# DefaultRui/VLN-VER

Measured on AMD Instinct MI355X. Metric: viewpoints/sec (multi-view->voxel fwd+bwd), vocc.py config, higher is better.
Workload: dtype bf16

## Files before the change

### vln-ver_amd/csrc/ver_common.h

```cpp
#pragma once
#include <hip/hip_runtime.h>
#include <stdint.h>
#include "../../include/ver_ops.h"

#define VER_WAVE 64

int ver_fail(int code, const char* fmt, ...);
int ver_check_launch(const char* what);
int ver_zero_async(void* ptr, size_t bytes, void* stream);

#define VER_REQUIRE(cond, code, ...)                     \
    do {                                                 \
        if (!(cond)) return ver_fail(code, __VA_ARGS__); \
    } while (0)

struct Bilinear {
    float w[4];
    int key[4];
    float gx[4];
    float gy[4];
    bool any;
};

template <bool GRAD>
// ... 109 lines not shown
```

### vln-ver_amd/csrc/ver_gemm.hip

```cpp
#include "ver_common.h"

namespace {
typedef __bf16 bf16x8 __attribute__((ext_vector_type(8)));
typedef float f32x16 __attribute__((ext_vector_type(16)));
typedef int i32x2 __attribute__((ext_vector_type(2)));
typedef int i32x4 __attribute__((ext_vector_type(4)));
typedef __attribute__((address_space(3))) void lds_void;

constexpr int kTile = 256;
constexpr int kStageBytes = 32768;
constexpr int kStages = 4;
constexpr int kLdsBytes = kStages * kStageBytes;

template <int OFF>
__device__ __forceinline__ i32x2 tr_read(int addr) {
    i32x2 v;
    asm volatile("ds_read_b64_tr_b16 %0, %1 offset:%2" : "=v"(v) : "v"(addr), "n"(OFF) : "memory");
    return v;
}
template <int OFF>
__device__ __forceinline__ i32x4 row_read(int addr) {
    i32x4 v;
    asm volatile("ds_read_b128 %0, %1 offset:%2" : "=v"(v) : "v"(addr), "n"(OFF) : "memory");
    return v;
// ... 12 lines not shown
    int CW, ncst;
    signed char kind[64], dz[64], dy[64], dx[64];
    signed char pl[64];
    long plane_elems;
};

struct GemmArgs {
    const __bf16* A;
    const __bf16* W;
    const float* bias;
    __bf16* C;
    long lda, ldw, ldc, M;
    int K, N, tiles_n, T, per_xcd;
    int S, Kc;
    float* ws;
    TapArgs t;
};

struct GemmLane {
    int offA0, offA1;
    int offB0, offB1;
    int voA, voW;
    int stepW;
    int stepA16;
    int dmaA, dmaW;
};

constexpr int kOutside = (int)0x80000000;
template <int L>
__device__ __forceinline__ int cell_off(const TapArgs& t, int b, int zl, int y, int x, int dz) {
// ... 57 lines not shown
            __builtin_amdgcn_raw_ptr_buffer_load_lds(rcst, (lds_void*)(dst + 1024), 16, tl.vo2, ch, 0, 0);
        } else {
            __builtin_amdgcn_raw_ptr_buffer_load_lds(ra, (lds_void*)dst, 16, tl.vo1, ch, 0, 0);
            __builtin_amdgcn_raw_ptr_buffer_load_lds(ra, (lds_void*)(dst + 1024), 16, tl.vo2, ch, 0, 0);
        }
        tl.ch = ch + 64;
        if (tl.ch == __builtin_amdgcn_readfirstlane(tl.seglen)) {
            tl.ch = 0;
            tl.tap = __builtin_amdgcn_readfirstlane(tl.tap) + 1;
            tap_offsets<IMPL>(t, tl, ra);
        }
    }
}


template <int ST, int IMPL>
__device__ __forceinline__ void phase(char* lds, f32x16 (&acc)[4][2], const GemmLane& c, __amdgpu_buffer_rsrc_t& ra,
                                      __amdgpu_buffer_rsrc_t rw, int& soA, int& soW, const TapArgs& t, TapLane& tl,
                                      __amdgpu_buffer_rsrc_t rcst) {
    constexpr int SB = (ST & 1) * kStageBytes;
    constexpr int UP = ST >= 2 ? 65536 : 0;
    const int a0 = c.offA0 + UP, a1 = c.offA1 + UP, b0 = c.offB0 + UP, b1 = c.offB1 + UP;
    i32x4 av[2][4];
    i32x2 bl[2][2], bh[2][2];
    av[0][0] = row_read<SB>(a0);
    av[0][1] = row_read<SB + 2048>(a0);
    bl[0][0] = tr_read<SB + 16384>(b0);
    bh[0][0] = tr_read<SB + 16384 + 512>(b0);
    bl[0][1] = tr_read<SB + 16384>(b1);
    bh[0][1] = tr_read<SB + 16384 + 512>(b1);
    av[0][2] = row_read<SB + 4096>(a0);
    av[0][3] = row_read<SB + 6144>(a0);
    av[1][0] = row_read<SB>(a1);
    av[1][1] = row_read<SB + 2048>(a1);
    bl[1][0] = tr_read<SB + 24576>(b0);
    bh[1][0] = tr_read<SB + 24576 + 512>(b0);
    bl[1][1] = tr_read<SB + 24576>(b1);
    bh[1][1] = tr_read<SB + 24576 + 512>(b1);
    av[1][2] = row_read<SB + 4096>(a1);
    av[1][3] = row_read<SB + 6144>(a1);
    constexpr int DS = ((ST + 2) % kStages) * kStageBytes;
    request_a<IMPL>(lds + DS + c.dmaA, c, ra, rcst, soA, t, tl);
    __builtin_amdgcn_raw_ptr_buffer_load_lds(rw, (lds_void*)(lds + DS + 16384 + c.dmaW), 16, c.voW, soW, 0, 0);
    __builtin_amdgcn_raw_ptr_buffer_load_lds(rw, (lds_void*)(lds + DS + 24576 + c.dmaW), 16, c.voW, soW + c.stepW, 0, 0);
    soW += 2 * c.stepW;
    asm volatile("s_waitcnt vmcnt(4)" ::: "memory");
    __builtin_amdgcn_s_barrier();
    asm volatile("s_waitcnt lgkmcnt(0)"
                 : "+v"(av[0][0]), "+v"(av[0][1]), "+v"(av[0][2]), "+v"(av[0][3]), "+v"(av[1][0]), "+v"(av[1][1]), "+v"(av[1][2]),
                   "+v"(av[1][3]), "+v"(bl[0][0]), "+v"(bh[0][0]), "+v"(bl[0][1]), "+v"(bh[0][1]), "+v"(bl[1][0]), "+v"(bh[1][0]),
                   "+v"(bl[1][1]), "+v"(bh[1][1])
                 :
                 : "memory");
    bf16x8 a[2][4], b[2][2];
#pragma unroll
    for (int u = 0; u < 2; ++u) {
#pragma unroll
        for (int i = 0; i < 4; ++i) a[u][i] = __builtin_bit_cast(bf16x8, av[u][i]);
        b[u][0] = frag(bl[u][0], bh[u][0]);
        b[u][1] = frag(bl[u][1], bh[u][1]);
    }
    __builtin_amdgcn_sched_barrier(0);
    __builtin_amdgcn_s_setprio(1);
#pragma unroll
    for (int u = 0; u < 2; ++u)
#pragma unroll
        for (int it = 0; it < 4; ++it)
#pragma unroll
            for (int jt = 0; jt < 2; ++jt)
                acc[it][jt] = __builtin_amdgcn_mfma_f32_32x32x16_bf16(a[u][it], b[u][jt], acc[it][jt], 0, 0, 0);
    __builtin_amdgcn_s_setprio(0);
    __builtin_amdgcn_sched_barrier(0);
    __builtin_amdgcn_s_barrier();
}

template <int IMPL>
__global__ __launch_bounds__(512) void k_gemm_nn(GemmArgs p) {
    extern __shared__ __attribute__((aligned(1024))) char lds[];
    const int tid = threadIdx.x, lane = tid & 63;
    const int wave = __builtin_amdgcn_readfirstlane(tid >> 6);
    const int wr = wave >> 2, wc = wave & 3;
    const int item = (int)(blockIdx.x & 7) * p.per_xcd + (int)(blockIdx.x >> 3);
    if ((int)(blockIdx.x >> 3) >= p.per_xcd || item >= p.T * p.S) return;
    const int split = item / p.T, tile = item - split * p.T;
    const int mt = tile / p.tiles_n, nt = tile - mt * p.tiles_n;
    const long row0 = (long)mt * kTile;
    const int k0 = split * p.Kc, klen = min(p.Kc, p.K - k0);
    const int nphase = klen / 32;

    const __bf16* ab = IMPL < 0 ? p.A + row0 * p.lda + k0 : p.t.lattice;
    const long abytes = IMPL < 0 ? ((p.M - row0 - 1) * p.lda + klen) * 2 : p.t.lattice_bytes;
    __amdgpu_buffer_rsrc_t ra = __builtin_amdgcn_make_buffer_rsrc((void*)ab, 0, (int)max(0L, min(abytes, 0xFFFFFFFFL)), 0x00020000);
    const __amdgpu_buffer_rsrc_t rcst = __builtin_amdgcn_make_buffer_rsrc((void*)(IMPL < 0 ? ab : p.t.cst), 0,
                                                                          (int)(IMPL < 0 ? 0L : max(0L, min(p.t.cst_bytes, 0x7FFFFFFFL))), 0x00020000);
    const __bf16* wb = p.W + (long)k0 * p.ldw + (long)nt * kTile;
    const long wbytes = ((long)(klen - 1) * p.ldw + p.N - (long)nt * kTile) * 2;
    const __amdgpu_buffer_rsrc_t rw = __builtin_amdgcn_make_buffer_rsrc((void*)wb, 0, (int)max(0L, min(wbytes, 0xFFFFFFFFL)), 0x00020000);
    GemmLane c;
    {
        const int prow = 32 * wave + (lane >> 2);
        const int pch = (lane & 3) ^ ((prow >> 2) & 3);
        c.voA = (int)(prow * p.lda * 2) + pch * 16;
        c.dmaA = wave * 2048;
        c.stepA16 = (int)(16 * p.lda * 2);
        const int wrow = lane >> 3, wch = (lane & 7) ^ (((wrow >> 1) & 1) << 2);
        c.voW = (int)(((8 * (wave >> 2) + wrow) * p.ldw + 64 * (wave & 3)) * 2) + wch * 16;
        c.stepW = (int)(16 * p.ldw * 2);
        c.dmaW = wave * 1024;
    }
    {
        const int lbase = (int)(uintptr_t)(__attribute__((address_space(3))) char*)lds;
        const int i = lane & 31, sw = (i >> 2) & 3;
        c.offA0 = lbase + (128 * wr + i) * 64 + (((lane >> 5) ^ sw) << 4);
        c.offA1 = c.offA0 ^ 32;
        const int q = lane >> 4, cl = lane & 15;
        const int lowch = (2 * (q & 1) + ((cl & 3) >> 1)) ^ (((cl >> 3) & 1) << 2);
        c.offB0 = lbase + ((q >> 1) * 32 + (cl >> 2)) * 128 + lowch * 16 + (cl & 1) * 8 + wc * 1024;
        c.offB1 = c.offB0 ^ 64;
    }
    TapLane tl = {};
    if constexpr (IMPL >= 0) {
        const int prow = 32 * wave + (lane >> 2);
        const int hw = p.t.H * p.t.W;
        auto decode = [&](long r, int& b, int& zl, int& y, int& x) {
            if (r >= p.M) {
                b = -1, zl = y = x = 0;
                return;
            }
            b = (int)(r / p.t.P);
            const int pos = (int)(r - (long)b * p.t.P);
            zl = pos / hw;
            const int rem = pos - zl * hw;
            y = rem / p.t.W;
            x = rem - y * p.t.W;
        };
        decode(row0 + prow, tl.b1, tl.zl1, tl.y1, tl.x1);
        decode(row0 + prow + 16, tl.b2, tl.zl2, tl.y2, tl.x2);
        tl.pos1 = (tl.zl1 * p.t.H + tl.y1) * p.t.W + tl.x1;
        tl.pos2 = (tl.zl2 * p.t.H + tl.y2) * p.t.W + tl.x2;
        tl.chunk = ((lane & 3) ^ ((prow >> 2) & 3)) * 16;
        tl.tap = 0, tl.ch = 0;
        tap_offsets<IMPL>(p.t, tl, ra);
    }
    f32x16 acc[4][2];
#pragma unroll
    for (int it = 0; it < 4; ++it)
#pragma unroll
        for (int jt = 0; jt < 2; ++jt)
#pragma unroll
            for (int r = 0; r < 16; ++r) acc[it][jt][r] = 0.0f;

    int soA = 0, soW = 0;
#pragma unroll
    for (int s = 0; s < 2; ++s) {
        request_a<IMPL>(lds + s * kStageBytes + c.dmaA, c, ra, rcst, soA, p.t, tl);
        __builtin_amdgcn_raw_ptr_buffer_load_lds(rw, (lds_void*)(lds + s * kStageBytes + 16384 + c.dmaW), 16, c.voW, soW, 0, 0);
        __builtin_amdgcn_raw_ptr_buffer_load_lds(rw, (lds_void*)(lds + s * kStageBytes + 24576 + c.dmaW), 16, c.voW, soW + c.stepW, 0, 0);
        soW += 2 * c.stepW;
    }
    asm volatile("s_waitcnt vmcnt(4)" ::: "memory");
    __builtin_amdgcn_s_barrier();
    if (wr == 1) __builtin_amdgcn_s_barrier();

    int s = 0;
    for (; s + kStages <= nphase; s += kStages) {
        phase<0, IMPL>(lds, acc, c, ra, rw, soA, soW, p.t, tl, rcst);
        phase<1, IMPL>(lds, acc, c, ra, rw, soA, soW, p.t, tl, rcst);
        phase<2, IMPL>(lds, acc, c, ra, rw, soA, soW, p.t, tl, rcst);
        phase<3, IMPL>(lds, acc, c, ra, rw, soA, soW, p.t, tl, rcst);
    }
    const int rem = nphase - s;
    if (rem > 0) phase<0, IMPL>(lds, acc, c, ra, rw, soA, soW, p.t, tl, rcst);
    if (rem > 1) phase<1, IMPL>(lds, acc, c, ra, rw, soA, soW, p.t, tl, rcst);
    if (rem > 2) phase<2, IMPL>(lds, acc, c, ra, rw, soA, soW, p.t, tl, rcst);
    if (wr == 0) __builtin_amdgcn_s_barrier();
    asm volatile("s_waitcnt vmcnt(0)" ::: "memory");

    if (p.S > 1) {
        float* out = p.ws + (long)split * p.M * p.N;
        const long i0 = row0 + 128 * wr + 4 * (lane >> 5);
        const int j0 = nt * kTile + 64 * wc + (lane & 31);
#pragma unroll
        for (int it = 0; it < 4; ++it)
#pragma unroll
            for (int jt = 0; jt < 2; ++jt) {
                const int j = j0 + 32 * jt;
#pragma unroll
                for (int r = 0; r < 16; ++r) {
                    const long i = i0 + 32 * it + (r & 3) + 8 * (r >> 2);
                    if (i < p.M && j < p.N) out[i * p.N + j] = acc[it][jt][r];
                }
            }
        return;
    }
    __bf16* cb = p.C + row0 * p.ldc + (long)nt * kTile;
    const long cbytes = ((p.M - row0 - 1) * p.ldc + p.N - (long)nt * kTile) * 2;
    const __amdgpu_buffer_rsrc_t rc = __builtin_amdgcn_make_buffer_rsrc((void*)cb, 0, (int)max(0L, min(cbytes, 0xFFFFFFFFL)), 0x00020000);
    const int ldc2 = (int)(p.ldc * 2);
    const int vbase = (128 * wr + 4 * (lane >> 5)) * ldc2 + (64 * wc + (lane & 31)) * 2;
    const bool haspos = IMPL >= 0 && p.t.rowpos != nullptr;
    const int pos0 = haspos ? (int)((row0 + 128 * wr + 4 * (lane >> 5)) % p.t.P) : 0;
#pragma unroll
    for (int jt = 0; jt < 2; ++jt) {
        const int j = nt * kTile + 64 * wc + 32 * jt + (lane & 31);
        const float bj = (p.bias && j < p.N) ? p.bias[j] : 0.0f;
        const int vo = j < p.N ? vbase + 64 * jt : -2;
#pragma unroll
        for (int it = 0; it < 4; ++it) {
            float add[16];
#pragma unroll
            for (int r = 0; r < 16; ++r) {
                add[r] = bj;
                if (haspos) {
                    int pp = pos0 + 32 * it + (r & 3) + 8 * (r >> 2);
                    while (pp >= p.t.P) pp -= p.t.P;
                    const long row = row0 + 128 * wr + 4 * (lane >> 5) + 32 * it + (r & 3) + 8 * (r >> 2);
                    if (j < p.N && row < p.M) add[r] += p.t.rowpos[(long)pp * p.N + j];
                }
            }
#pragma unroll
            for (int r = 0; r < 16; ++r) {
                const __bf16 v = (__bf16)(acc[it][jt][r] + add[r]);
                __builtin_amdgcn_raw_buffer_store_b16(__builtin_bit_cast(short, v), rc, vo, (32 * it + (r & 3) + 8 * (r >> 2)) * ldc2, 0);
            }
        }
    }
}
__global__ __launch_bounds__(256) void k_gemm_reduce(const float* __restrict__ ws, const float* __restrict__ bias,
                                                     __bf16* __restrict__ c, long ldc, int S, long M, int N) {
    const long n4 = M * N / 4;
    const long stride = M * N;
    for (long e = blockIdx.x * 256L + threadIdx.x; e < n4; e += (long)gridDim.x * 256) {
        float4 acc = *reinterpret_cast<const float4*>(ws + 4 * e);
        for (int s = 1; s < S; ++s) {
            const float4 v = *reinterpret_cast<const float4*>(ws + s * stride + 4 * e);
            acc.x += v.x, acc.y += v.y, acc.z += v.z, acc.w += v.w;
        }
        const long i = (4 * e) / N;
        const int j = (int)(4 * e - i * N);
        if (bias) acc.x += bias[j], acc.y += bias[j + 1], acc.z += bias[j + 2], acc.w += bias[j + 3];
        typedef __bf16 bf16x4 __attribute__((ext_vector_type(4)));
// ... 49 lines not shown
    p.W = (const __bf16*)w;
    p.bias = bias;
    p.C = (__bf16*)c;
    p.lda = lda;
    p.ldw = ldw;
    p.ldc = ldc;
    p.M = M;
    p.K = K;
    p.N = N;
    p.tiles_n = (N + kTile - 1) / kTile;
    p.T = (int)((M + kTile - 1) / kTile) * p.tiles_n;
    p.Kc = splits == 1 ? K : ((K + splits - 1) / splits + 31) / 32 * 32;
    p.S = splits == 1 ? 1 : (K + p.Kc - 1) / p.Kc;
    p.ws = (float*)workspace;
    p.per_xcd = (p.T * p.S + 7) / 8;
    p.t = TapArgs{};
    hipError_t e = hipFuncSetAttribute((const void*)k_gemm_nn<-1>, hipFuncAttributeMaxDynamicSharedMemorySize, kLdsBytes);
    if (e != hipSuccess) return ver_fail(VER_ELAUNCH, "ver_gemm_nn: LDS attribute: %s", hipGetErrorString(e));
    hipLaunchKernelGGL(k_gemm_nn<-1>, dim3((unsigned)(8 * p.per_xcd)), dim3(512), kLdsBytes, st, p);
    if (p.S > 1) {
        long grid = (M * N / 4 + 255) / 256;
        if (grid > 4096) grid = 4096;
        hipLaunchKernelGGL(k_gemm_reduce, dim3((unsigned)grid), dim3(256), 0, st, (const float*)workspace, bias, (__bf16*)c, ldc, p.S, M, N);
    }
    return ver_check_launch("ver_gemm_nn");
}

extern "C" int ver_gemm_nn_segments(const void* lattice, int layout, int B, int H, int W, int C, const int* taps, int ntaps,
                                    const void* cst, int ncst, int cw, const void* w, long ldw, const float* rowpos,
                                    const float* bias, void* c, long ldc, int N, void* stream);
// ... 46 lines not shown
    p.W = (const __bf16*)w;
    p.bias = bias;
    p.C = (__bf16*)c;
    p.lda = 0;
    p.ldw = ldw;
    p.ldc = ldc;
    p.M = M;
    p.K = (int)K;
    p.N = N;
    p.tiles_n = (N + kTile - 1) / kTile;
    p.T = (int)((M + kTile - 1) / kTile) * p.tiles_n;
    p.Kc = (int)K;
    p.S = 1;
    p.ws = nullptr;
    p.per_xcd = (p.T + 7) / 8;
    p.t = TapArgs{};
    p.t.lattice = (const __bf16*)lattice;
    p.t.lattice_bytes = lbytes;
    p.t.B = B, p.t.H = H, p.t.W = W, p.t.C = C, p.t.ntaps = ntaps, p.t.P = 2 * H * W;
    p.t.rowpos = rowpos;
    VER_REQUIRE((plane_elems == 0) == (tap_plane == nullptr) && plane_elems >= 0 && (plane_elems == 0 || (nplanes > 0 && nplanes <= 64 &&
                plane_elems % 8 == 0)), VER_EINVAL, "ver_gemm_nn_planes: plane_elems, nplanes and tap_plane come together");
    p.t.plane_elems = plane_elems;
    for (int i = 0; i < ntaps; ++i) {
        VER_REQUIRE(!tap_plane || (tap_plane[i] >= 0 && tap_plane[i] < nplanes), VER_EINVAL, "ver_gemm_nn_planes: tap %d reads plane %d of %d", i,
                    tap_plane ? tap_plane[i] : 0, nplanes);
        p.t.pl[i] = (signed char)(tap_plane ? tap_plane[i] : 0);
    }
    p.t.cst = (const __bf16*)cst;
    p.t.cst_bytes = cst ? (long)2 * H * W * ncst * cw * 2 : 0;
// ... 25 lines not shown
```

### vln-ver_amd/csrc/ver_wgrad.hip

```cpp
#include <cstdlib>
#include "ver_common.h"

namespace {
typedef __bf16 bf16x8 __attribute__((ext_vector_type(8)));
typedef float f32x16 __attribute__((ext_vector_type(16)));
typedef short s16x4 __attribute__((ext_vector_type(4)));
typedef short s16x8 __attribute__((ext_vector_type(8)));
typedef __attribute__((address_space(3))) s16x4 lds_s16x4;
typedef __attribute__((address_space(3))) void lds_void;

constexpr int kTile = 256;
constexpr int kSlabRows = 16;
constexpr int kSlabBytes = 2 * kSlabRows * kTile * 2;
constexpr int kRing = 8;
constexpr int kLdsBytes = kRing * kSlabBytes;

typedef int i32x2 __attribute__((ext_vector_type(2)));
typedef int i32x4 __attribute__((ext_vector_type(4)));

template <int OFF>
__device__ __forceinline__ i32x2 tr_read(int addr) {
    i32x2 v;
    asm volatile("ds_read_b64_tr_b16 %0, %1 offset:%2" : "=v"(v) : "v"(addr), "n"(OFF) : "memory");
    return v;
// ... 5 lines not shown
struct WgradArgs {
    const __bf16* A;
    const __bf16* G;
    float* ws;
    long lda, ldg, M, Mc;
    int S, Ka, N, tiles_n, T;
    void* out;
    long ldo;
    int out_bf16;
    const __bf16* lattice;
    long lattice_bytes;
    const __bf16* cst;
    long cst_bytes;
    int B, H, W, C, P, CW, ncst, nseg;
    int seg_start[65];
    signed char kind[64], dz[64], dy[64], dx[64];
};

constexpr int kOutsideW = (int)0x80000000;
template <int L>
__device__ __forceinline__ int wcell_off(const WgradArgs& t, int b, int zl, int y, int x, int dz) {
    if ((unsigned)y >= (unsigned)t.H || (unsigned)x >= (unsigned)t.W) return kOutsideW;
    const int j = dz >> 1;
    int v;
    if (L == 0)
        v = ((b * 4 + zl + dz) * t.H + y) * t.W + x;
    else if (L == 2)
        v = ((((b * 2 + zl) * t.H + y) * t.W + x) << 1) + j;
    else
        v = (((((((y & 1) << 1 | (x & 1)) * t.B + b) * 2 + zl) * (t.H >> 1) + (y >> 1)) * (t.W >> 1) + (x >> 1)) << 1) + j;
// ... 30 lines not shown
    tl.boff += tl.pend;
    tl.rows_left -= kSlabRows;
    tl.vo = tl.rows_left > 0 ? (int)((unsigned)tfetched + (unsigned)tl.boff) : kOutsideW;
    tl.taddr += 4 * kSlabRows;
    tl.pend = 0;
    if (tl.taddr >= tl.tend) tl.taddr -= 4 * t.P, tl.pend = tl.bstep;
}

struct WgradLane {
    int offA0, offA1, offB0, offB1;
    int voA, voG;
    int stepA, stepG;
    int dmaoff;
};

template <int SLOT>
__device__ __forceinline__ void read_slab(const WgradLane& c, i32x2 (&al)[4], i32x2 (&ah)[4], i32x2 (&bl)[2], i32x2 (&bh)[2]) {
    constexpr int SB = (SLOT & 3) * kSlabBytes;
    constexpr int UP = SLOT >= 4 ? 65536 : 0;
    const int a0 = c.offA0 + UP, a1 = c.offA1 + UP, b0 = c.offB0 + UP, b1 = c.offB1 + UP;
    al[0] = tr_read<SB>(a0);
    ah[0] = tr_read<SB + 512>(a0);
    bl[0] = tr_read<SB>(b0);
    bh[0] = tr_read<SB + 512>(b0);
    al[1] = tr_read<SB>(a1);
    ah[1] = tr_read<SB + 512>(a1);
    bl[1] = tr_read<SB>(b1);
    bh[1] = tr_read<SB + 512>(b1);
    al[2] = tr_read<SB + 1024>(a0);
    ah[2] = tr_read<SB + 1536>(a0);
    al[3] = tr_read<SB + 1024>(a1);
    ah[3] = tr_read<SB + 1536>(a1);
}

template <int PS, int KP, int PF, int IMPL>
__device__ __forceinline__ void phase(char* lds, f32x16 (&acc)[4][2], const WgradLane& c, __amdgpu_buffer_rsrc_t ra,
                                      __amdgpu_buffer_rsrc_t rg, unsigned& soA, unsigned& soG, const WgradArgs& t, WTapLane& tl) {
    i32x2 al[KP][4], ah[KP][4], bl[KP][2], bh[KP][2];
    int tnext = 0;
    read_slab<PS * KP>(c, al[0], ah[0], bl[0], bh[0]);
    if constexpr (KP == 2) read_slab<PS * KP + 1>(c, al[KP - 1], ah[KP - 1], bl[KP - 1], bh[KP - 1]);
#pragma unroll
    for (int u = 0; u < KP; ++u) {
        const int ds = (PS * KP + u + PF) % kRing;
        if constexpr (IMPL < 0) {
            __builtin_amdgcn_raw_ptr_buffer_load_lds(ra, (lds_void*)(lds + ds * kSlabBytes + c.dmaoff), 16, c.voA, (int)soA, 0, 0);
        } else {
            static_assert(IMPL < 0 || KP == 1, "implicit A: one slab per phase");
            __builtin_amdgcn_raw_ptr_buffer_load_lds(ra, (lds_void*)(lds + ds * kSlabBytes + c.dmaoff), 16, tl.vo, 0, 0, 0);
            tnext = lds_read_b32(tl.taddr);
        }
        __builtin_amdgcn_raw_ptr_buffer_load_lds(rg, (lds_void*)(lds + ds * kSlabBytes + kSlabBytes / 2 + c.dmaoff), 16, c.voG, (int)soG, 0, 0);
        soA += (unsigned)c.stepA;
        soG += (unsigned)c.stepG;
    }
    asm volatile("s_waitcnt vmcnt(%0)" ::"n"(2 * (PF - KP)) : "memory");
    __builtin_amdgcn_s_barrier();
    asm volatile("s_waitcnt lgkmcnt(0)"
                 : "+v"(al[0][0]), "+v"(ah[0][0]), "+v"(al[0][1]), "+v"(ah[0][1]), "+v"(al[0][2]), "+v"(ah[0][2]), "+v"(al[0][3]),
                   "+v"(ah[0][3]), "+v"(bl[0][0]), "+v"(bh[0][0]), "+v"(bl[0][1]), "+v"(bh[0][1]), "+v"(tnext)
                 :
                 : "memory");

    if constexpr (KP == 2)
        asm volatile(""
                     : "+v"(al[KP - 1][0]), "+v"(ah[KP - 1][0]), "+v"(al[KP - 1][1]), "+v"(ah[KP - 1][1]), "+v"(al[KP - 1][2]),
                       "+v"(ah[KP - 1][2]), "+v"(al[KP - 1][3]), "+v"(ah[KP - 1][3]), "+v"(bl[KP - 1][0]), "+v"(bh[KP - 1][0]),
                       "+v"(bl[KP - 1][1]), "+v"(bh[KP - 1][1])
                     :
                     : "memory");
    bf16x8 a[KP][4], b[KP][2];
#pragma unroll
    for (int u = 0; u < KP; ++u) {
#pragma unroll
        for (int i = 0; i < 4; ++i) a[u][i] = frag(al[u][i], ah[u][i]);
        b[u][0] = frag(bl[u][0], bh[u][0]);
        b[u][1] = frag(bl[u][1], bh[u][1]);
    }
    __builtin_amdgcn_sched_barrier(0);
    __builtin_amdgcn_s_setprio(1);
#pragma unroll
    for (int u = 0; u < KP; ++u)
#pragma unroll
        for (int it = 0; it < 4; ++it)
#pragma unroll
            for (int jt = 0; jt < 2; ++jt)
                acc[it][jt] = __builtin_amdgcn_mfma_f32_32x32x16_bf16(a[u][it], b[u][jt], acc[it][jt], 0, 0, 0);
    __builtin_amdgcn_s_setprio(0);
    __builtin_amdgcn_sched_barrier(0);
    if constexpr (IMPL >= 0) {
        wtap_step(t, tl, tnext);
        __builtin_amdgcn_sched_barrier(0);
    }
    __builtin_amdgcn_s_barrier();
}

template <int PS, int KP, int PF, int IMPL>
__device__ __forceinline__ void phases_from(int left, char* lds, f32x16 (&acc)[4][2], const WgradLane& c,
                                            __amdgpu_buffer_rsrc_t ra, __amdgpu_buffer_rsrc_t rg, unsigned& soA, unsigned& soG,
                                            const WgradArgs& t, WTapLane& tl) {
    if constexpr (PS < kRing / KP) {
        if (left > PS * KP) {
            phase<PS, KP, PF, IMPL>(lds, acc, c, ra, rg, soA, soG, t, tl);
            phases_from<PS + 1, KP, PF, IMPL>(left, lds, acc, c, ra, rg, soA, soG, t, tl);
        }
    }
}

template <int KP, int PF, int IMPL>
__device__ __forceinline__ void wgrad_body(const WgradArgs& p) {
    static_assert(PF >= KP && PF + (KP == 1 ? 2 : 4) <= kRing, "prefetch distance against the ring (WAR on the slot)");
    extern __shared__ __attribute__((aligned(1024))) char lds[];
    const int tid = threadIdx.x, lane = tid & 63;
    const int wave = __builtin_amdgcn_readfirstlane(tid >> 6);
    const int wr = wave >> 2, wc = wave & 3;
    int chunk, tile;
    {
        const int b = blockIdx.x;
        if ((p.S & 7) == 0) {
            const int xcd = b & 7, idx = b >> 3;
            chunk = xcd + 8 * (idx / p.T);
            tile = idx % p.T;
        } else {
            chunk = b / p.T;
            tile = b % p.T;
        }
    }
    const int mt = tile / p.tiles_n, nt = tile - mt * p.tiles_n;
    const long row0 = (long)chunk * p.Mc;
    const long rows = max(0L, min(p.Mc, p.M - row0));
    const int nslab = (int)((rows + kSlabRows * KP - 1) / (kSlabRows * KP)) * KP;

    const __bf16* ab = IMPL < 0 ? p.A + row0 * p.lda + (long)mt * kTile : nullptr;
    const __bf16* gb = p.G + row0 * p.ldg + (long)nt * kTile;
    const long abytes = ((p.M - row0 - 1) * p.lda + p.Ka - (long)mt * kTile) * 2;
    const long gbytes = ((p.M - row0 - 1) * p.ldg + p.N - (long)nt * kTile) * 2;
    const __amdgpu_buffer_rsrc_t rg = __builtin_amdgcn_make_buffer_rsrc((void*)gb, 0, (int)max(0L, min(gbytes, 0xFFFFFFFFL)), 0x00020000);
    WgradLane c;
    const int prow = lane >> 3, pch = (lane & 7) ^ (((prow >> 1) & 1) << 2);
    WTapLane tl = {};
    bool a_cst = false;
    if constexpr (IMPL >= 0) {
// ... 29 lines not shown
        IMPL < 0 ? __builtin_amdgcn_make_buffer_rsrc((void*)ab, 0, (int)max(0L, min(abytes, 0xFFFFFFFFL)), 0x00020000)
                 : __builtin_amdgcn_make_buffer_rsrc((void*)(a_cst ? p.cst : p.lattice), 0,
                                                     (int)max(0L, min(a_cst ? p.cst_bytes : p.lattice_bytes, 0x7FFFFFFFL)), 0x00020000);
    c.voA = (int)(((8 * (wave >> 2) + prow) * p.lda + 64 * (wave & 3)) * 2) + pch * 16;
    c.voG = (int)(((8 * (wave >> 2) + prow) * p.ldg + 64 * (wave & 3)) * 2) + pch * 16;
    c.stepA = (int)(kSlabRows * p.lda * 2);
    c.stepG = (int)(kSlabRows * p.ldg * 2);
    c.dmaoff = wave * 1024;
    unsigned soA = 0, soG = 0;

    {
        const int q = lane >> 4, cl = lane & 15;
        const int lowch = (2 * (q & 1) + ((cl & 3) >> 1)) ^ (((cl >> 3) & 1) << 2);
        const int lbase = (int)(uintptr_t)(__attribute__((address_space(3))) char*)lds;
        const int rowoff = lbase + ((q >> 1) * 32 + (cl >> 2)) * 128 + lowch * 16 + (cl & 1) * 8;
        c.offA0 = rowoff + 2 * wr * 1024;
        c.offA1 = c.offA0 ^ 64;
        c.offB0 = rowoff + wc * 1024 + kSlabBytes / 2;
        c.offB1 = c.offB0 ^ 64;
    }

    f32x16 acc[4][2];
#pragma unroll
    for (int it = 0; it < 4; ++it)
#pragma unroll
        for (int jt = 0; jt < 2; ++jt)
#pragma unroll
            for (int r = 0; r < 16; ++r) acc[it][jt][r] = 0.0f;

#pragma unroll
    for (int s = 0; s < PF; ++s) {
        if constexpr (IMPL < 0) {
            __builtin_amdgcn_raw_ptr_buffer_load_lds(ra, (lds_void*)(lds + s * kSlabBytes + c.dmaoff), 16, c.voA, (int)soA, 0, 0);
        } else {
            __builtin_amdgcn_raw_ptr_buffer_load_lds(ra, (lds_void*)(lds + s * kSlabBytes + c.dmaoff), 16, tl.vo, 0, 0, 0);
            int tn = lds_read_b32(tl.taddr);
            asm volatile("s_waitcnt lgkmcnt(0)" : "+v"(tn)::"memory");
            wtap_step(p, tl, tn);
        }
        __builtin_amdgcn_raw_ptr_buffer_load_lds(rg, (lds_void*)(lds + s * kSlabBytes + kSlabBytes / 2 + c.dmaoff), 16, c.voG, (int)soG, 0, 0);
        soA += (unsigned)c.stepA;
        soG += (unsigned)c.stepG;
    }
    asm volatile("s_waitcnt vmcnt(%0)" ::"n"(2 * (PF - KP)) : "memory");
    __builtin_amdgcn_s_barrier();
    if (wr == 1) __builtin_amdgcn_s_barrier();

    int s = 0;
    for (; s + kRing <= nslab; s += kRing) phases_from<0, KP, PF, IMPL>(kRing, lds, acc, c, ra, rg, soA, soG, p, tl);
    phases_from<0, KP, PF, IMPL>(nslab - s, lds, acc, c, ra, rg, soA, soG, p, tl);
    if (wr == 0) __builtin_amdgcn_s_barrier();
    asm volatile("s_waitcnt vmcnt(0)" ::: "memory");

    const int i0 = mt * kTile + 128 * wr + 4 * (lane >> 5), j0 = nt * kTile + 64 * wc + (lane & 31);
    if (p.S == 1 && p.out) {
#pragma unroll
        for (int it = 0; it < 4; ++it)
#pragma unroll
            for (int jt = 0; jt < 2; ++jt) {
                const int j = j0 + 32 * jt;
#pragma unroll
                for (int r = 0; r < 16; ++r) {
                    const int i = i0 + 32 * it + (r & 3) + 8 * (r >> 2);
                    if (i < p.Ka && j < p.N) {
                        if (p.out_bf16)
                            reinterpret_cast<__bf16*>(p.out)[(long)i * p.ldo + j] = (__bf16)acc[it][jt][r];
                        else
                            reinterpret_cast<float*>(p.out)[(long)i * p.ldo + j] = acc[it][jt][r];
                    }
                }
            }
        return;
    }
    float* out = p.ws + (long)chunk * p.Ka * p.N;
#pragma unroll
    for (int it = 0; it < 4; ++it)
#pragma unroll
        for (int jt = 0; jt < 2; ++jt) {
            const int j = j0 + 32 * jt;
#pragma unroll
            for (int r = 0; r < 16; ++r) {
                const int i = i0 + 32 * it + (r & 3) + 8 * (r >> 2);
                if (i < p.Ka && j < p.N) out[(long)i * p.N + j] = acc[it][jt][r];
            }
        }
}

template <int KP, int PF>
__global__ __launch_bounds__(512) void k_wgrad_tn(WgradArgs p) {
    wgrad_body<KP, PF, -1>(p);
}

template <int L, int PF>
__global__ __launch_bounds__(512) void k_wgrad_tn_seg(WgradArgs p) {
    wgrad_body<1, PF, L>(p);
}

template <typename OT>
__global__ __launch_bounds__(256) void k_wgrad_reduce(const float* __restrict__ ws, OT* __restrict__ out, long ldo, int S,
                                                      int Ka, int N) {
    const long n4 = (long)Ka * N / 4;
    const long stride = (long)Ka * N;
    for (long e = blockIdx.x * 256L + threadIdx.x; e < n4; e += (long)gridDim.x * 256) {
        float4 acc = *reinterpret_cast<const float4*>(ws + 4 * e);
        for (int s = 1; s < S; ++s) {
            const float4 v = *reinterpret_cast<const float4*>(ws + s * stride + 4 * e);
            acc.x += v.x;
            acc.y += v.y;
            acc.z += v.z;
            acc.w += v.w;
// ... 111 lines not shown
    p.G = (const __bf16*)g;
    p.ws = (float*)workspace;
    p.lda = lda;
    p.ldg = ldg;
    p.M = M;
    p.Mc = Mc;
    p.S = S;
    p.Ka = Ka;
    p.N = N;
    p.tiles_n = (N + kTile - 1) / kTile;
    p.T = ((Ka + kTile - 1) / kTile) * p.tiles_n;
    const bool direct = S == 1 && M > 0;
    p.out = direct ? out : nullptr;
    p.ldo = ldo;
    p.out_bf16 = out_dtype == VER_BF16;
    hipError_t e = hipSuccess;
    if (M > 0) {
        switch (flags & 15) {
            case 4: launch_tn<1, 4>(p, p.T * S, st, e); break;
            case 5: launch_tn<1, 5>(p, p.T * S, st, e); break;
            case 6: launch_tn<1, 6>(p, p.T * S, st, e); break;
            case 8 + 2: launch_tn<2, 2>(p, p.T * S, st, e); break;
            case 8 + 4: launch_tn<2, 4>(p, p.T * S, st, e); break;
            default: launch_tn<1, 3>(p, p.T * S, st, e); break;
        }
        if (e != hipSuccess) return ver_fail(VER_ELAUNCH, "ver_wgrad_tn: LDS attribute: %s", hipGetErrorString(e));
    } else if (int zrc = ver_zero_async(workspace, (size_t)S * Ka * N * sizeof(float), st)) {
        return zrc;
    }
    if (direct) return ver_check_launch("ver_wgrad_tn");
// ... 103 lines not shown
```

Measured before the change: 701.8.

## Specialize GEMM and wgrad kernels for ragged edge tiles to skip dead MFMAs

Adds NIT-templated variants of the bf16 GEMM and weight-gradient tile bodies that compute only 1, 2 or 4 row sub-tiles per wave. Edge tiles with at most 64 valid columns or at most 128 valid rows now dispatch to the reduced variant, which drops LDS reads and MFMAs on padding. Wave-to-row and column mappings are remapped so the waves still cover the valid region. The path is on by default and can be turned off with VER_RAGGED_TILES=0. The cost is more kernel code paths, possible register and instruction-cache pressure, and waves that may sit idle or duplicate work in the reduced modes.

Measured after the change: 705.8 (median of 6 runs). No clear change (+0.6%).

```diff
diff --git a/vln-ver_amd/csrc/ver_common.h b/vln-ver_amd/csrc/ver_common.h
--- a/vln-ver_amd/csrc/ver_common.h
+++ b/vln-ver_amd/csrc/ver_common.h
@@ -1,6 +1,7 @@
 #pragma once
 #include <hip/hip_runtime.h>
 #include <stdint.h>
+#include <stdlib.h>
 #include "../../include/ver_ops.h"
 
 #define VER_WAVE 64
@@ -8,6 +9,11 @@
 int ver_fail(int code, const char* fmt, ...);
 int ver_check_launch(const char* what);
 int ver_zero_async(void* ptr, size_t bytes, void* stream);
+
+static inline int ver_ragged_tiles() {
+    const char* v = getenv("VER_RAGGED_TILES");
+    return !(v && v[0] == '0' && v[1] == 0);
+}
 
 #define VER_REQUIRE(cond, code, ...)                     \
     do {                                                 \
diff --git a/vln-ver_amd/csrc/ver_gemm.hip b/vln-ver_amd/csrc/ver_gemm.hip
--- a/vln-ver_amd/csrc/ver_gemm.hip
+++ b/vln-ver_amd/csrc/ver_gemm.hip
@@ -50,6 +50,7 @@
     int K, N, tiles_n, T, per_xcd;
     int S, Kc;
     float* ws;
+    int ragged;
     TapArgs t;
 };
 
@@ -137,31 +138,35 @@
 }
 
 
-template <int ST, int IMPL>
-__device__ __forceinline__ void phase(char* lds, f32x16 (&acc)[4][2], const GemmLane& c, __amdgpu_buffer_rsrc_t& ra,
+template <int ST, int IMPL, int NIT>
+__device__ __forceinline__ void phase(char* lds, f32x16 (&acc)[NIT][2], const GemmLane& c, __amdgpu_buffer_rsrc_t& ra,
                                       __amdgpu_buffer_rsrc_t rw, int& soA, int& soW, const TapArgs& t, TapLane& tl,
                                       __amdgpu_buffer_rsrc_t rcst) {
     constexpr int SB = (ST & 1) * kStageBytes;
     constexpr int UP = ST >= 2 ? 65536 : 0;
     const int a0 = c.offA0 + UP, a1 = c.offA1 + UP, b0 = c.offB0 + UP, b1 = c.offB1 + UP;
-    i32x4 av[2][4];
+    i32x4 av[2][NIT];
     i32x2 bl[2][2], bh[2][2];
     av[0][0] = row_read<SB>(a0);
-    av[0][1] = row_read<SB + 2048>(a0);
+    if constexpr (NIT >= 2) av[0][1] = row_read<SB + 2048>(a0);
     bl[0][0] = tr_read<SB + 16384>(b0);
     bh[0][0] = tr_read<SB + 16384 + 512>(b0);
     bl[0][1] = tr_read<SB + 16384>(b1);
     bh[0][1] = tr_read<SB + 16384 + 512>(b1);
-    av[0][2] = row_read<SB + 4096>(a0);
-    av[0][3] = row_read<SB + 6144>(a0);
+    if constexpr (NIT == 4) {
+        av[0][2] = row_read<SB + 4096>(a0);
+        av[0][3] = row_read<SB + 6144>(a0);
+    }
     av[1][0] = row_read<SB>(a1);
-    av[1][1] = row_read<SB + 2048>(a1);
+    if constexpr (NIT >= 2) av[1][1] = row_read<SB + 2048>(a1);
     bl[1][0] = tr_read<SB + 24576>(b0);
     bh[1][0] = tr_read<SB + 24576 + 512>(b0);
     bl[1][1] = tr_read<SB + 24576>(b1);
     bh[1][1] = tr_read<SB + 24576 + 512>(b1);
-    av[1][2] = row_read<SB + 4096>(a1);
-    av[1][3] = row_read<SB + 6144>(a1);
+    if constexpr (NIT == 4) {
+        av[1][2] = row_read<SB + 4096>(a1);
+        av[1][3] = row_read<SB + 6144>(a1);
+    }
     constexpr int DS = ((ST + 2) % kStages) * kStageBytes;
     request_a<IMPL>(lds + DS + c.dmaA, c, ra, rcst, soA, t, tl);
     __builtin_amdgcn_raw_ptr_buffer_load_lds(rw, (lds_void*)(lds + DS + 16384 + c.dmaW), 16, c.voW, soW, 0, 0);
@@ -169,17 +174,30 @@
     soW += 2 * c.stepW;
     asm volatile("s_waitcnt vmcnt(4)" ::: "memory");
     __builtin_amdgcn_s_barrier();
-    asm volatile("s_waitcnt lgkmcnt(0)"
-                 : "+v"(av[0][0]), "+v"(av[0][1]), "+v"(av[0][2]), "+v"(av[0][3]), "+v"(av[1][0]), "+v"(av[1][1]), "+v"(av[1][2]),
-                   "+v"(av[1][3]), "+v"(bl[0][0]), "+v"(bh[0][0]), "+v"(bl[0][1]), "+v"(bh[0][1]), "+v"(bl[1][0]), "+v"(bh[1][0]),
-                   "+v"(bl[1][1]), "+v"(bh[1][1])
-                 :
-                 : "memory");
-    bf16x8 a[2][4], b[2][2];
+    if constexpr (NIT == 4)
+        asm volatile("s_waitcnt lgkmcnt(0)"
+                     : "+v"(av[0][0]), "+v"(av[0][1]), "+v"(av[0][2]), "+v"(av[0][3]), "+v"(av[1][0]), "+v"(av[1][1]), "+v"(av[1][2]),
+                       "+v"(av[1][3]), "+v"(bl[0][0]), "+v"(bh[0][0]), "+v"(bl[0][1]), "+v"(bh[0][1]), "+v"(bl[1][0]), "+v"(bh[1][0]),
+                       "+v"(bl[1][1]), "+v"(bh[1][1])
+                     :
+                     : "memory");
+    else if constexpr (NIT == 2)
+        asm volatile("s_waitcnt lgkmcnt(0)"
+                     : "+v"(av[0][0]), "+v"(av[0][1]), "+v"(av[1][0]), "+v"(av[1][1]), "+v"(bl[0][0]), "+v"(bh[0][0]), "+v"(bl[0][1]),
+                       "+v"(bh[0][1]), "+v"(bl[1][0]), "+v"(bh[1][0]), "+v"(bl[1][1]), "+v"(bh[1][1])
+                     :
+                     : "memory");
+    else
+        asm volatile("s_waitcnt lgkmcnt(0)"
+                     : "+v"(av[0][0]), "+v"(av[1][0]), "+v"(bl[0][0]), "+v"(bh[0][0]), "+v"(bl[0][1]), "+v"(bh[0][1]), "+v"(bl[1][0]),
+                       "+v"(bh[1][0]), "+v"(bl[1][1]), "+v"(bh[1][1])
+                     :
+                     : "memory");
+    bf16x8 a[2][NIT], b[2][2];
 #pragma unroll
     for (int u = 0; u < 2; ++u) {
 #pragma unroll
-        for (int i = 0; i < 4; ++i) a[u][i] = __builtin_bit_cast(bf16x8, av[u][i]);
+        for (int i = 0; i < NIT; ++i) a[u][i] = __builtin_bit_cast(bf16x8, av[u][i]);
         b[u][0] = frag(bl[u][0], bh[u][0]);
         b[u][1] = frag(bl[u][1], bh[u][1]);
     }
@@ -188,7 +206,7 @@
 #pragma unroll
     for (int u = 0; u < 2; ++u)
 #pragma unroll
-        for (int it = 0; it < 4; ++it)
+        for (int it = 0; it < NIT; ++it)
 #pragma unroll
             for (int jt = 0; jt < 2; ++jt)
                 acc[it][jt] = __builtin_amdgcn_mfma_f32_32x32x16_bf16(a[u][it], b[u][jt], acc[it][jt], 0, 0, 0);
@@ -197,16 +215,14 @@
     __builtin_amdgcn_s_barrier();
 }
 
-template <int IMPL>
-__global__ __launch_bounds__(512) void k_gemm_nn(GemmArgs p) {
+template <int IMPL, int NIT>
+__device__ __forceinline__ void gemm_tile(const GemmArgs& p, int split, int mt, int nt) {
     extern __shared__ __attribute__((aligned(1024))) char lds[];
     const int tid = threadIdx.x, lane = tid & 63;
     const int wave = __builtin_amdgcn_readfirstlane(tid >> 6);
     const int wr = wave >> 2, wc = wave & 3;
-    const int item = (int)(blockIdx.x & 7) * p.per_xcd + (int)(blockIdx.x >> 3);
-    if ((int)(blockIdx.x >> 3) >= p.per_xcd || item >= p.T * p.S) return;
-    const int split = item / p.T, tile = item - split * p.T;
-    const int mt = tile / p.tiles_n, nt = tile - mt * p.tiles_n;
+    const int rbase = NIT == 4 ? 128 * wr : NIT == 2 ? 64 * wr : 128 * wr + 32 * wc;
+    const int cblk = NIT == 1 ? 0 : wc;
     const long row0 = (long)mt * kTile;
     const int k0 = split * p.Kc, klen = min(p.Kc, p.K - k0);
     const int nphase = klen / 32;
@@ -234,11 +250,11 @@
     {
         const int lbase = (int)(uintptr_t)(__attribute__((address_space(3))) char*)lds;
         const int i = lane & 31, sw = (i >> 2) & 3;
-        c.offA0 = lbase + (128 * wr + i) * 64 + (((lane >> 5) ^ sw) << 4);
+        c.offA0 = lbase + (rbase + i) * 64 + (((lane >> 5) ^ sw) << 4);
         c.offA1 = c.offA0 ^ 32;
         const int q = lane >> 4, cl = lane & 15;
         const int lowch = (2 * (q & 1) + ((cl & 3) >> 1)) ^ (((cl >> 3) & 1) << 2);
-        c.offB0 = lbase + ((q >> 1) * 32 + (cl >> 2)) * 128 + lowch * 16 + (cl & 1) * 8 + wc * 1024;
+        c.offB0 = lbase + ((q >> 1) * 32 + (cl >> 2)) * 128 + lowch * 16 + (cl & 1) * 8 + cblk * 1024;
         c.offB1 = c.offB0 ^ 64;
     }
     TapLane tl = {};
@@ -265,9 +281,9 @@
         tl.tap = 0, tl.ch = 0;
         tap_offsets<IMPL>(p.t, tl, ra);
     }
-    f32x16 acc[4][2];
-#pragma unroll
-    for (int it = 0; it < 4; ++it)
+    f32x16 acc[NIT][2];
+#pragma unroll
+    for (int it = 0; it < NIT; ++it)
 #pragma unroll
         for (int jt = 0; jt < 2; ++jt)
 #pragma unroll
@@ -287,24 +303,24 @@
 
     int s = 0;
     for (; s + kStages <= nphase; s += kStages) {
-        phase<0, IMPL>(lds, acc, c, ra, rw, soA, soW, p.t, tl, rcst);
-        phase<1, IMPL>(lds, acc, c, ra, rw, soA, soW, p.t, tl, rcst);
-        phase<2, IMPL>(lds, acc, c, ra, rw, soA, soW, p.t, tl, rcst);
-        phase<3, IMPL>(lds, acc, c, ra, rw, soA, soW, p.t, tl, rcst);
+        phase<0, IMPL, NIT>(lds, acc, c, ra, rw, soA, soW, p.t, tl, rcst);
+        phase<1, IMPL, NIT>(lds, acc, c, ra, rw, soA, soW, p.t, tl, rcst);
+        phase<2, IMPL, NIT>(lds, acc, c, ra, rw, soA, soW, p.t, tl, rcst);
+        phase<3, IMPL, NIT>(lds, acc, c, ra, rw, soA, soW, p.t, tl, rcst);
     }
     const int rem = nphase - s;
-    if (rem > 0) phase<0, IMPL>(lds, acc, c, ra, rw, soA, soW, p.t, tl, rcst);
-    if (rem > 1) phase<1, IMPL>(lds, acc, c, ra, rw, soA, soW, p.t, tl, rcst);
-    if (rem > 2) phase<2, IMPL>(lds, acc, c, ra, rw, soA, soW, p.t, tl, rcst);
+    if (rem > 0) phase<0, IMPL, NIT>(lds, acc, c, ra, rw, soA, soW, p.t, tl, rcst);
+    if (rem > 1) phase<1, IMPL, NIT>(lds, acc, c, ra, rw, soA, soW, p.t, tl, rcst);
+    if (rem > 2) phase<2, IMPL, NIT>(lds, acc, c, ra, rw, soA, soW, p.t, tl, rcst);
     if (wr == 0) __builtin_amdgcn_s_barrier();
     asm volatile("s_waitcnt vmcnt(0)" ::: "memory");
 
     if (p.S > 1) {
         float* out = p.ws + (long)split * p.M * p.N;
-        const long i0 = row0 + 128 * wr + 4 * (lane >> 5);
-        const int j0 = nt * kTile + 64 * wc + (lane & 31);
-#pragma unroll
-        for (int it = 0; it < 4; ++it)
+        const long i0 = row0 + rbase + 4 * (lane >> 5);
+        const int j0 = nt * kTile + 64 * cblk + (lane & 31);
+#pragma unroll
+        for (int it = 0; it < NIT; ++it)
 #pragma unroll
             for (int jt = 0; jt < 2; ++jt) {
                 const int j = j0 + 32 * jt;
@@ -320,16 +336,16 @@
     const long cbytes = ((p.M - row0 - 1) * p.ldc + p.N - (long)nt * kTile) * 2;
     const __amdgpu_buffer_rsrc_t rc = __builtin_amdgcn_make_buffer_rsrc((void*)cb, 0, (int)max(0L, min(cbytes, 0xFFFFFFFFL)), 0x00020000);
     const int ldc2 = (int)(p.ldc * 2);
-    const int vbase = (128 * wr + 4 * (lane >> 5)) * ldc2 + (64 * wc + (lane & 31)) * 2;
+    const int vbase = (rbase + 4 * (lane >> 5)) * ldc2 + (64 * cblk + (lane & 31)) * 2;
     const bool haspos = IMPL >= 0 && p.t.rowpos != nullptr;
-    const int pos0 = haspos ? (int)((row0 + 128 * wr + 4 * (lane >> 5)) % p.t.P) : 0;
+    const int pos0 = haspos ? (int)((row0 + rbase + 4 * (lane >> 5)) % p.t.P) : 0;
 #pragma unroll
     for (int jt = 0; jt < 2; ++jt) {
-        const int j = nt * kTile + 64 * wc + 32 * jt + (lane & 31);
+        const int j = nt * kTile + 64 * cblk + 32 * jt + (lane & 31);
         const float bj = (p.bias && j < p.N) ? p.bias[j] : 0.0f;
         const int vo = j < p.N ? vbase + 64 * jt : -2;
 #pragma unroll
-        for (int it = 0; it < 4; ++it) {
+        for (int it = 0; it < NIT; ++it) {
             float add[16];
 #pragma unroll
             for (int r = 0; r < 16; ++r) {
@@ -337,7 +353,7 @@
                 if (haspos) {
                     int pp = pos0 + 32 * it + (r & 3) + 8 * (r >> 2);
                     while (pp >= p.t.P) pp -= p.t.P;
-                    const long row = row0 + 128 * wr + 4 * (lane >> 5) + 32 * it + (r & 3) + 8 * (r >> 2);
+                    const long row = row0 + rbase + 4 * (lane >> 5) + 32 * it + (r & 3) + 8 * (r >> 2);
                     if (j < p.N && row < p.M) add[r] += p.t.rowpos[(long)pp * p.N + j];
                 }
             }
@@ -348,6 +364,19 @@
             }
         }
     }
+}
+
+template <int IMPL>
+__global__ __launch_bounds__(512) void k_gemm_nn(GemmArgs p) {
+    const int item = (int)(blockIdx.x & 7) * p.per_xcd + (int)(blockIdx.x >> 3);
+    if ((int)(blockIdx.x >> 3) >= p.per_xcd || item >= p.T * p.S) return;
+    const int split = item / p.T, tile = item - split * p.T;
+    const int mt = tile / p.tiles_n, nt = tile - mt * p.tiles_n;
+    if constexpr (IMPL < 0) {
+        if (p.ragged && p.N - nt * kTile <= 64) return gemm_tile<IMPL, 1>(p, split, mt, nt);
+        if (p.ragged && p.M - (long)mt * kTile <= 128) return gemm_tile<IMPL, 2>(p, split, mt, nt);
+    }
+    gemm_tile<IMPL, 4>(p, split, mt, nt);
 }
 __global__ __launch_bounds__(256) void k_gemm_reduce(const float* __restrict__ ws, const float* __restrict__ bias,
                                                      __bf16* __restrict__ c, long ldc, int S, long M, int N) {
@@ -427,6 +456,7 @@
     p.S = splits == 1 ? 1 : (K + p.Kc - 1) / p.Kc;
     p.ws = (float*)workspace;
     p.per_xcd = (p.T * p.S + 7) / 8;
+    p.ragged = ver_ragged_tiles();
     p.t = TapArgs{};
     hipError_t e = hipFuncSetAttribute((const void*)k_gemm_nn<-1>, hipFuncAttributeMaxDynamicSharedMemorySize, kLdsBytes);
     if (e != hipSuccess) return ver_fail(VER_ELAUNCH, "ver_gemm_nn: LDS attribute: %s", hipGetErrorString(e));
@@ -503,6 +533,7 @@
     p.S = 1;
     p.ws = nullptr;
     p.per_xcd = (p.T + 7) / 8;
+    p.ragged = 0;
     p.t = TapArgs{};
     p.t.lattice = (const __bf16*)lattice;
     p.t.lattice_bytes = lbytes;
diff --git a/vln-ver_amd/csrc/ver_wgrad.hip b/vln-ver_amd/csrc/ver_wgrad.hip
--- a/vln-ver_amd/csrc/ver_wgrad.hip
+++ b/vln-ver_amd/csrc/ver_wgrad.hip
@@ -43,6 +43,7 @@
     long cst_bytes;
     int B, H, W, C, P, CW, ncst, nseg;
     int seg_start[65];
+    int ragged;
     signed char kind[64], dz[64], dy[64], dx[64];
 };
 
@@ -103,8 +104,8 @@
     int dmaoff;
 };
 
-template <int SLOT>
-__device__ __forceinline__ void read_slab(const WgradLane& c, i32x2 (&al)[4], i32x2 (&ah)[4], i32x2 (&bl)[2], i32x2 (&bh)[2]) {
+template <int SLOT, int NIT>
+__device__ __forceinline__ void read_slab(const WgradLane& c, i32x2 (&al)[NIT], i32x2 (&ah)[NIT], i32x2 (&bl)[2], i32x2 (&bh)[2]) {
     constexpr int SB = (SLOT & 3) * kSlabBytes;
     constexpr int UP = SLOT >= 4 ? 65536 : 0;
     const int a0 = c.offA0 + UP, a1 = c.offA1 + UP, b0 = c.offB0 + UP, b1 = c.offB1 + UP;
@@ -112,23 +113,27 @@
     ah[0] = tr_read<SB + 512>(a0);
     bl[0] = tr_read<SB>(b0);
     bh[0] = tr_read<SB + 512>(b0);
-    al[1] = tr_read<SB>(a1);
-    ah[1] = tr_read<SB + 512>(a1);
+    if constexpr (NIT >= 2) {
+        al[1] = tr_read<SB>(a1);
+        ah[1] = tr_read<SB + 512>(a1);
+    }
     bl[1] = tr_read<SB>(b1);
     bh[1] = tr_read<SB + 512>(b1);
-    al[2] = tr_read<SB + 1024>(a0);
-    ah[2] = tr_read<SB + 1536>(a0);
-    al[3] = tr_read<SB + 1024>(a1);
-    ah[3] = tr_read<SB + 1536>(a1);
-}
-
-template <int PS, int KP, int PF, int IMPL>
-__device__ __forceinline__ void phase(char* lds, f32x16 (&acc)[4][2], const WgradLane& c, __amdgpu_buffer_rsrc_t ra,
+    if constexpr (NIT == 4) {
+        al[2] = tr_read<SB + 1024>(a0);
+        ah[2] = tr_read<SB + 1536>(a0);
+        al[3] = tr_read<SB + 1024>(a1);
+        ah[3] = tr_read<SB + 1536>(a1);
+    }
+}
+
+template <int PS, int KP, int PF, int IMPL, int NIT>
+__device__ __forceinline__ void phase(char* lds, f32x16 (&acc)[NIT][2], const WgradLane& c, __amdgpu_buffer_rsrc_t ra,
                                       __amdgpu_buffer_rsrc_t rg, unsigned& soA, unsigned& soG, const WgradArgs& t, WTapLane& tl) {
-    i32x2 al[KP][4], ah[KP][4], bl[KP][2], bh[KP][2];
+    i32x2 al[KP][NIT], ah[KP][NIT], bl[KP][2], bh[KP][2];
     int tnext = 0;
-    read_slab<PS * KP>(c, al[0], ah[0], bl[0], bh[0]);
-    if constexpr (KP == 2) read_slab<PS * KP + 1>(c, al[KP - 1], ah[KP - 1], bl[KP - 1], bh[KP - 1]);
+    read_slab<PS * KP, NIT>(c, al[0], ah[0], bl[0], bh[0]);
+    if constexpr (KP == 2) read_slab<PS * KP + 1, NIT>(c, al[KP - 1], ah[KP - 1], bl[KP - 1], bh[KP - 1]);
 #pragma unroll
     for (int u = 0; u < KP; ++u) {
         const int ds = (PS * KP + u + PF) % kRing;
@@ -145,24 +150,40 @@
     }
     asm volatile("s_waitcnt vmcnt(%0)" ::"n"(2 * (PF - KP)) : "memory");
     __builtin_amdgcn_s_barrier();
-    asm volatile("s_waitcnt lgkmcnt(0)"
-                 : "+v"(al[0][0]), "+v"(ah[0][0]), "+v"(al[0][1]), "+v"(ah[0][1]), "+v"(al[0][2]), "+v"(ah[0][2]), "+v"(al[0][3]),
-                   "+v"(ah[0][3]), "+v"(bl[0][0]), "+v"(bh[0][0]), "+v"(bl[0][1]), "+v"(bh[0][1]), "+v"(tnext)
-                 :
-                 : "memory");
-
-    if constexpr (KP == 2)
-        asm volatile(""
-                     : "+v"(al[KP - 1][0]), "+v"(ah[KP - 1][0]), "+v"(al[KP - 1][1]), "+v"(ah[KP - 1][1]), "+v"(al[KP - 1][2]),
-                       "+v"(ah[KP - 1][2]), "+v"(al[KP - 1][3]), "+v"(ah[KP - 1][3]), "+v"(bl[KP - 1][0]), "+v"(bh[KP - 1][0]),
-                       "+v"(bl[KP - 1][1]), "+v"(bh[KP - 1][1])
+    if constexpr (NIT == 4) {
+        asm volatile("s_waitcnt lgkmcnt(0)"
+                     : "+v"(al[0][0]), "+v"(ah[0][0]), "+v"(al[0][1]), "+v"(ah[0][1]), "+v"(al[0][2]), "+v"(ah[0][2]), "+v"(al[0][3]),
+                       "+v"(ah[0][3]), "+v"(bl[0][0]), "+v"(bh[0][0]), "+v"(bl[0][1]), "+v"(bh[0][1]), "+v"(tnext)
                      :
                      : "memory");
-    bf16x8 a[KP][4], b[KP][2];
+
+        if constexpr (KP == 2)
+            asm volatile(""
+                         : "+v"(al[KP - 1][0]), "+v"(ah[KP - 1][0]), "+v"(al[KP - 1][1]), "+v"(ah[KP - 1][1]), "+v"(al[KP - 1][2]),
+                           "+v"(ah[KP - 1][2]), "+v"(al[KP - 1][3]), "+v"(ah[KP - 1][3]), "+v"(bl[KP - 1][0]), "+v"(bh[KP - 1][0]),
+                           "+v"(bl[KP - 1][1]), "+v"(bh[KP - 1][1])
+                         :
+                         : "memory");
+    } else {
+        asm volatile("s_waitcnt lgkmcnt(0)"
+                     : "+v"(al[0][0]), "+v"(ah[0][0]), "+v"(bl[0][0]), "+v"(bh[0][0]), "+v"(bl[0][1]), "+v"(bh[0][1]), "+v"(tnext)
+                     :
+                     : "memory");
+        if constexpr (NIT == 2) asm volatile("" : "+v"(al[0][NIT - 1]), "+v"(ah[0][NIT - 1])::"memory");
+        if constexpr (KP == 2) {
+            asm volatile(""
+                         : "+v"(al[KP - 1][0]), "+v"(ah[KP - 1][0]), "+v"(bl[KP - 1][0]), "+v"(bh[KP - 1][0]), "+v"(bl[KP - 1][1]),
+                           "+v"(bh[KP - 1][1])
+                         :
+                         : "memory");
+            if constexpr (NIT == 2) asm volatile("" : "+v"(al[KP - 1][NIT - 1]), "+v"(ah[KP - 1][NIT - 1])::"memory");
+        }
+    }
+    bf16x8 a[KP][NIT], b[KP][2];
 #pragma unroll
     for (int u = 0; u < KP; ++u) {
 #pragma unroll
-        for (int i = 0; i < 4; ++i) a[u][i] = frag(al[u][i], ah[u][i]);
+        for (int i = 0; i < NIT; ++i) a[u][i] = frag(al[u][i], ah[u][i]);
         b[u][0] = frag(bl[u][0], bh[u][0]);
         b[u][1] = frag(bl[u][1], bh[u][1]);
     }
@@ -171,7 +192,7 @@
 #pragma unroll
     for (int u = 0; u < KP; ++u)
 #pragma unroll
-        for (int it = 0; it < 4; ++it)
+        for (int it = 0; it < NIT; ++it)
 #pragma unroll
             for (int jt = 0; jt < 2; ++jt)
                 acc[it][jt] = __builtin_amdgcn_mfma_f32_32x32x16_bf16(a[u][it], b[u][jt], acc[it][jt], 0, 0, 0);
@@ -184,37 +205,38 @@
     __builtin_amdgcn_s_barrier();
 }
 
-template <int PS, int KP, int PF, int IMPL>
-__device__ __forceinline__ void phases_from(int left, char* lds, f32x16 (&acc)[4][2], const WgradLane& c,
+template <int PS, int KP, int PF, int IMPL, int NIT>
+__device__ __forceinline__ void phases_from(int left, char* lds, f32x16 (&acc)[NIT][2], const WgradLane& c,
                                             __amdgpu_buffer_rsrc_t ra, __amdgpu_buffer_rsrc_t rg, unsigned& soA, unsigned& soG,
                                             const WgradArgs& t, WTapLane& tl) {
     if constexpr (PS < kRing / KP) {
         if (left > PS * KP) {
-            phase<PS, KP, PF, IMPL>(lds, acc, c, ra, rg, soA, soG, t, tl);
-            phases_from<PS + 1, KP, PF, IMPL>(left, lds, acc, c, ra, rg, soA, soG, t, tl);
-        }
-    }
-}
-
-template <int KP, int PF, int IMPL>
-__device__ __forceinline__ void wgrad_body(const WgradArgs& p) {
+            phase<PS, KP, PF, IMPL, NIT>(lds, acc, c, ra, rg, soA, soG, t, tl);
+            phases_from<PS + 1, KP, PF, IMPL, NIT>(left, lds, acc, c, ra, rg, soA, soG, t, tl);
+        }
+    }
+}
+
+__device__ __forceinline__ void wgrad_item(const WgradArgs& p, int& chunk, int& tile) {
+    const int b = blockIdx.x;
+    if ((p.S & 7) == 0) {
+        const int xcd = b & 7, idx = b >> 3;
+        chunk = xcd + 8 * (idx / p.T);
+        tile = idx % p.T;
+    } else {
+        chunk = b / p.T;
+        tile = b % p.T;
+    }
+}
+
+template <int KP, int PF, int IMPL, int NIT>
+__device__ __forceinline__ void wgrad_body(const WgradArgs& p, int chunk, int tile) {
     static_assert(PF >= KP && PF + (KP == 1 ? 2 : 4) <= kRing, "prefetch distance against the ring (WAR on the slot)");
+    static_assert(IMPL < 0 || NIT == 4, "implicit A: full tiles only");
     extern __shared__ __attribute__((aligned(1024))) char lds[];
     const int tid = threadIdx.x, lane = tid & 63;
     const int wave = __builtin_amdgcn_readfirstlane(tid >> 6);
     const int wr = wave >> 2, wc = wave & 3;
-    int chunk, tile;
-    {
-        const int b = blockIdx.x;
-        if ((p.S & 7) == 0) {
-            const int xcd = b & 7, idx = b >> 3;
-            chunk = xcd + 8 * (idx / p.T);
-            tile = idx % p.T;
-        } else {
-            chunk = b / p.T;
-            tile = b % p.T;
-        }
-    }
     const int mt = tile / p.tiles_n, nt = tile - mt * p.tiles_n;
     const long row0 = (long)chunk * p.Mc;
     const long rows = max(0L, min(p.Mc, p.M - row0));
@@ -274,15 +296,17 @@
         const int lowch = (2 * (q & 1) + ((cl & 3) >> 1)) ^ (((cl >> 3) & 1) << 2);
         const int lbase = (int)(uintptr_t)(__attribute__((address_space(3))) char*)lds;
         const int rowoff = lbase + ((q >> 1) * 32 + (cl >> 2)) * 128 + lowch * 16 + (cl & 1) * 8;
-        c.offA0 = rowoff + 2 * wr * 1024;
+        if constexpr (NIT == 4) c.offA0 = rowoff + 2 * wr * 1024;
+        else if constexpr (NIT == 2) c.offA0 = rowoff + wr * 1024;
+        else c.offA0 = (rowoff + (2 * wr + (wc >> 1)) * 1024) ^ ((wc & 1) << 6);
         c.offA1 = c.offA0 ^ 64;
-        c.offB0 = rowoff + wc * 1024 + kSlabBytes / 2;
+        c.offB0 = rowoff + (NIT == 1 ? 0 : wc) * 1024 + kSlabBytes / 2;
         c.offB1 = c.offB0 ^ 64;
     }
 
-    f32x16 acc[4][2];
-#pragma unroll
-    for (int it = 0; it < 4; ++it)
+    f32x16 acc[NIT][2];
+#pragma unroll
+    for (int it = 0; it < NIT; ++it)
 #pragma unroll
         for (int jt = 0; jt < 2; ++jt)
 #pragma unroll
@@ -307,15 +331,16 @@
     if (wr == 1) __builtin_amdgcn_s_barrier();
 
     int s = 0;
-    for (; s + kRing <= nslab; s += kRing) phases_from<0, KP, PF, IMPL>(kRing, lds, acc, c, ra, rg, soA, soG, p, tl);
-    phases_from<0, KP, PF, IMPL>(nslab - s, lds, acc, c, ra, rg, soA, soG, p, tl);
+    for (; s + kRing <= nslab; s += kRing) phases_from<0, KP, PF, IMPL, NIT>(kRing, lds, acc, c, ra, rg, soA, soG, p, tl);
+    phases_from<0, KP, PF, IMPL, NIT>(nslab - s, lds, acc, c, ra, rg, soA, soG, p, tl);
     if (wr == 0) __builtin_amdgcn_s_barrier();
     asm volatile("s_waitcnt vmcnt(0)" ::: "memory");
 
-    const int i0 = mt * kTile + 128 * wr + 4 * (lane >> 5), j0 = nt * kTile + 64 * wc + (lane & 31);
+    const int abase = NIT == 4 ? 128 * wr : NIT == 2 ? 64 * wr : 128 * wr + 32 * wc;
+    const int i0 = mt * kTile + abase + 4 * (lane >> 5), j0 = nt * kTile + 64 * (NIT == 1 ? 0 : wc) + (lane & 31);
     if (p.S == 1 && p.out) {
 #pragma unroll
-        for (int it = 0; it < 4; ++it)
+        for (int it = 0; it < NIT; ++it)
 #pragma unroll
             for (int jt = 0; jt < 2; ++jt) {
                 const int j = j0 + 32 * jt;
@@ -334,7 +359,7 @@
     }
     float* out = p.ws + (long)chunk * p.Ka * p.N;
 #pragma unroll
-    for (int it = 0; it < 4; ++it)
+    for (int it = 0; it < NIT; ++it)
 #pragma unroll
         for (int jt = 0; jt < 2; ++jt) {
             const int j = j0 + 32 * jt;
@@ -348,12 +373,19 @@
 
 template <int KP, int PF>
 __global__ __launch_bounds__(512) void k_wgrad_tn(WgradArgs p) {
-    wgrad_body<KP, PF, -1>(p);
+    int chunk, tile;
+    wgrad_item(p, chunk, tile);
+    const int mt = tile / p.tiles_n, nt = tile - mt * p.tiles_n;
+    if (p.ragged && p.N - nt * kTile <= 64) return wgrad_body<KP, PF, -1, 1>(p, chunk, tile);
+    if (p.ragged && p.Ka - mt * kTile <= 128) return wgrad_body<KP, PF, -1, 2>(p, chunk, tile);
+    wgrad_body<KP, PF, -1, 4>(p, chunk, tile);
 }
 
 template <int L, int PF>
 __global__ __launch_bounds__(512) void k_wgrad_tn_seg(WgradArgs p) {
-    wgrad_body<1, PF, L>(p);
+    int chunk, tile;
+    wgrad_item(p, chunk, tile);
+    wgrad_body<1, PF, L, 4>(p, chunk, tile);
 }
 
 template <typename OT>
@@ -495,6 +527,7 @@
     p.out = direct ? out : nullptr;
     p.ldo = ldo;
     p.out_bf16 = out_dtype == VER_BF16;
+    p.ragged = ver_ragged_tiles();
     hipError_t e = hipSuccess;
     if (M > 0) {
         switch (flags & 15) {
```
